# Chlumsky/msdfgen

Hardware: AMD Instinct MI355X
Metric: MSDF glyphs/sec (64x64, fp32) (higher is better)
Workload: dtype f64

## Files before the change

msdfgen_amd/csrc/msdf_cull.hpp:

```cpp
#pragma once

#include <string.h>
#include "msdf_device.hpp"

namespace msdfhip {

#define MSDF_CULL_SLACK (1.+1e-6)

MSDF_HD double cullUpperDistance(const EdgeRec &e, V2 c) {
    const V2 a = c-ld(e.p0), b = c-ld(e.pe), m = c-ld(e.mid);
    const double da = dot(a, a), db = dot(b, b), dm = dot(m, m);
    return sqrt(cmin(cmin(da, db), dm));
}

MSDF_HD float cullNearestSample2(const EdgeRec &e, V2 c) {
    const V2 a = c-ld(e.p0), b = c-ld(e.pe), m = c-ld(e.mid);
    return (float) cmin(cmin(dot(a, a), dot(b, b)), dot(m, m));
}
MSDF_HD float cullBumpUp(float f) {
    unsigned bits;
    memcpy(&bits, &f, sizeof(bits));
    if (bits < 0x7f800000u)
        ++bits;
    memcpy(&f, &bits, sizeof(bits));
    return f;
}
MSDF_HD float cullUpperFromSample2(float sample2) {
    return cullBumpUp(sqrtf(cullBumpUp(sample2)));
}

MSDF_HD double cullLowerDistance2(const EdgeRec &e, V2 c) {
    const double dx = cmax(cmax(e.lo[0]-c.x, c.x-e.hi[0]), 0.);
    const double dy = cmax(cmax(e.lo[1]-c.y, c.y-e.hi[1]), 0.);
    return dx*dx+dy*dy;
}

template <bool PERP>
MSDF_HD bool cullEdgeSurvives(const EdgeRec &e, V2 c, double r, double Umax) {
    const double R = r*MSDF_CULL_SLACK;
    const double reach = (Umax+R)*MSDF_CULL_SLACK;
    const double beyond = reach+R;
    if (!(cullLowerDistance2(e, c) > beyond*beyond))
        return true;
    if (PERP) {
        const V2 ap = c-ld(e.p0), aDir = ld(e.aDirN);
        const bool outsideA = dot(ap, ld(e.na))+R <= 0 || -dot(ap, aDir)+R <= 0;
        if (!outsideA && !(fabs(cross(ap, aDir))-R > reach))
            return true;
        const V2 bp = c-ld(e.pe), bDir = ld(e.bDirN);
        const bool outsideB = -dot(bp, ld(e.nb))+R <= 0 || dot(bp, bDir)+R <= 0;
        if (!outsideB && !(fabs(cross(bp, bDir))-R > reach))
            return true;
    }
    return false;
}

MSDF_HD unsigned cullOrderKeyOfSample2(float d2, int slot) {
    unsigned bits;
    memcpy(&bits, &d2, sizeof(bits));
    if (!(bits < 0x7f800000u))
        bits = 0x7f7ffff0u;
    return (bits&~15u)|(unsigned) (slot&15);
}
MSDF_HD unsigned cullOrderKey(const EdgeRec &e, V2 c, int slot) { return cullOrderKeyOfSample2(cullNearestSample2(e, c), slot); }
#define MSDF_CULL_KEY_DROPPED 0x7f800000u
#define MSDF_CULL_KEY_DROPPED_SEGMENTED 0xfffffff0u

template <int SEL>
MSDF_HD int cullMask(const EdgeRec &e) { return SEL <= 2 ? 1 : (e.color&7); }

}
```

msdfgen_amd/csrc/msdf_device.hpp:

```cpp
#pragma once

#include <stdint.h>
#include <stddef.h>
#include <math.h>
#include <float.h>

#if defined(__HIPCC__)
#define MSDF_HD __host__ __device__ inline
#define MSDF_NOINLINE __attribute__((noinline))
#define MSDF_NOUNROLL _Pragma("clang loop unroll(disable)")
#define MSDF_UNROLL _Pragma("unroll")
#if defined(__HIP_DEVICE_COMPILE__)
#define MSDF_UNIFORM(x) __builtin_amdgcn_readfirstlane(x)
#else
#define MSDF_UNIFORM(x) (x)
#endif
#else
#define MSDF_HD inline
#define MSDF_NOINLINE
#define MSDF_NOUNROLL
#define MSDF_UNROLL
#define MSDF_UNIFORM(x) (x)
#endif

#define MSDF_UNLIKELY(x) __builtin_expect(!!(x), 0)

#include "msdf_measure.hpp"

namespace msdfhip {

#if defined(__HIP_DEVICE_COMPILE__)
#define MSDF_WAVE_ANY(pred) (__any((int) (pred)) != 0)
#else
#define MSDF_WAVE_ANY(pred) (pred)
#endif


enum : int32_t {
    REC_A_ZERO = 1,
    REC_B_ZERO = 2,
    REC_NORMED = 4,
    REC_CORNER = 8,
    REC_FASTDIV = 16
};

struct V2 { double x, y; };

struct alignas(128) EdgeRec {
    double lo[2];
    double hi[2];
    double p0[2];
    double pe[2];
    double na[2];
    double nb[2];
    double aDirN[2];
    double bDirN[2];
    double ab[2];
    double k[6];
    double br[2];
    double ep0[2];
    double ep1[2];
    double e0dot;
    double e1dot;
    double rcp[4];
    double p1[2];
    double as_[2];
    double p2[2];
    double mid[2];
    int32_t type;
    int32_t color;
    int32_t flags;
    int32_t contour;
    double pad_[2];

    MSDF_HD V2 Lo() const; MSDF_HD V2 Hi() const; MSDF_HD V2 P0() const; MSDF_HD V2 PE() const; MSDF_HD V2 P1() const;
    MSDF_HD V2 NA() const; MSDF_HD V2 NB() const; MSDF_HD V2 ADirN() const; MSDF_HD V2 BDirN() const;
    MSDF_HD V2 AB() const; MSDF_HD V2 BR() const; MSDF_HD V2 AS() const; MSDF_HD V2 EP0() const; MSDF_HD V2 EP1() const;
    MSDF_HD double E0dot() const { return e0dot; }
    MSDF_HD double E1dot() const { return e1dot; }
    MSDF_HD double K(int i) const { return k[i]; }
    MSDF_HD double Rcp(int i) const { return rcp[i]; }
    MSDF_HD int Type() const { return type; }
    MSDF_HD int Color() const { return color; }
    MSDF_HD int Flags() const { return flags; }
};
static_assert(sizeof(EdgeRec) == 384, "EdgeRec layout");
static_assert(offsetof(EdgeRec, na) == 0x40 && offsetof(EdgeRec, ab) == 0x80 && offsetof(EdgeRec, br) == 0xc0 && offsetof(EdgeRec, rcp) == 0x100 &&
              offsetof(EdgeRec, p2) == 0x140 && offsetof(EdgeRec, type) == 0x160, "EdgeRec blocks");

MSDF_HD V2 mk(double x, double y) { V2 r; r.x = x; r.y = y; return r; }
MSDF_HD V2 operator+(V2 a, V2 b) { return mk(a.x+b.x, a.y+b.y); }
MSDF_HD V2 operator-(V2 a, V2 b) { return mk(a.x-b.x, a.y-b.y); }
MSDF_HD V2 operator-(V2 a) { return mk(-a.x, -a.y); }
MSDF_HD V2 operator*(double a, V2 b) { return mk(a*b.x, a*b.y); }
MSDF_HD double dot(V2 a, V2 b) { return a.x*b.x+a.y*b.y; }
MSDF_HD double cross(V2 a, V2 b) { return a.x*b.y-a.y*b.x; }

#if defined(__HIP_DEVICE_COMPILE__)
__device__ inline double leanSqrtCore(double x) {
    const double y = __builtin_amdgcn_rsq(x);
    double g = x*y;
    double h = y*.5;
    const double r = __builtin_fma(-h, g, .5);
    g = __builtin_fma(g, r, g);
    h = __builtin_fma(h, r, h);
    double d = __builtin_fma(-g, g, x);
    g = __builtin_fma(d, h, g);
    d = __builtin_fma(-g, g, x);
    return __builtin_fma(d, h, g);
}
__device__ inline double msdfSqrt(double x) {
    const unsigned hi = (unsigned) __double2hiint(x);
    if (__any((int) (hi-0x10000000u >= 0x7ff00000u-0x10000000u)))
        return sqrt(x);
    return leanSqrtCore(x);
}
#else
MSDF_HD double msdfSqrt(double x) { return sqrt(x); }
#endif
MSDF_HD double vlen(V2 a) { return msdfSqrt(a.x*a.x+a.y*a.y); }
MSDF_HD V2 ld(const double *p) { return mk(p[0], p[1]); }
MSDF_HD V2 EdgeRec::Lo() const { return ld(lo); }
MSDF_HD V2 EdgeRec::Hi() const { return ld(hi); }
MSDF_HD V2 EdgeRec::P0() const { return ld(p0); }
MSDF_HD V2 EdgeRec::PE() const { return ld(pe); }
MSDF_HD V2 EdgeRec::P1() const { return ld(p1); }
MSDF_HD V2 EdgeRec::NA() const { return ld(na); }
MSDF_HD V2 EdgeRec::NB() const { return ld(nb); }
MSDF_HD V2 EdgeRec::ADirN() const { return ld(aDirN); }
MSDF_HD V2 EdgeRec::BDirN() const { return ld(bDirN); }
MSDF_HD V2 EdgeRec::AB() const { return ld(ab); }
MSDF_HD V2 EdgeRec::BR() const { return ld(br); }
MSDF_HD V2 EdgeRec::AS() const { return ld(as_); }
MSDF_HD V2 EdgeRec::EP0() const { return ld(ep0); }
MSDF_HD V2 EdgeRec::EP1() const { return ld(ep1); }

MSDF_HD V2 normalize(V2 a, bool allowZero) {
    double len = vlen(a);
    if (len != 0)
        return mk(a.x/len, a.y/len);
    return mk(0, allowZero ? 0. : 1.);
}

MSDF_HD V2 normalizeLen(V2 a, double len, bool allowZero) {
    if (len != 0)
        return mk(a.x/len, a.y/len);
    return mk(0, allowZero ? 0. : 1.);
}

MSDF_HD V2 orthonormalFalse(V2 a) {
    double len = vlen(a);
    if (len != 0)
        return mk(a.y/len, -a.x/len);
    return mk(0, -1.);
}

MSDF_HD V2 mixv(V2 a, V2 b, double w) { return (1.-w)*a+w*b; }
MSDF_HD double nonZeroSign(double n) { return n > 0 ? 1. : -1.; }
MSDF_HD double dmin(double a, double b) { return b < a ? b : a; }
MSDF_HD double dmax(double a, double b) { return a < b ? b : a; }
MSDF_HD double cmax(double a, double b) { return __builtin_fmax(a, b); }
MSDF_HD double cmin(double a, double b) { return __builtin_fmin(a, b); }
MSDF_HD double median(double a, double b, double c) { return dmax(dmin(a, b), dmin(dmax(a, b), c)); }
MSDF_HD float fmin_(float a, float b) { return b < a ? b : a; }
MSDF_HD float fmax_(float a, float b) { return a < b ? b : a; }
MSDF_HD float medianf(float a, float b, float c) { return fmax_(fmin_(a, b), fmin_(fmax_(a, b), c)); }
MSDF_HD float med3Max(float a, float b) {
// ... 446 lines not shown
    if (o.neg > b.neg)
        b.neg = o.neg;
    if (o.pos < b.pos)
        b.pos = o.pos;
}

MSDF_HD double pbCompute(const PB &b) {
    double m = b.td < 0 ? b.neg : b.pos;
    if (pbHasNear(b) && fabs(b.perp) < fabs(m))
        m = b.perp;
    return m;
}

MSDF_HD bool getPerpendicularDistance(double &distance, V2 ep, V2 edgeDir) {
    double ts = dot(ep, edgeDir);
    if (ts > 0) {
        double perp = cross(ep, edgeDir);
        if (fabs(perp) < fabs(distance)) {
            distance = perp;
            return true;
        }
    }
    return false;
}

template <int SEL> struct SelTraits { enum { NPB = SEL == 1 ? 0 : SEL == 2 ? 1 : 3, NCH = SEL <= 2 ? 1 : SEL }; };

template <int SEL>
struct Selector {
    SD m;
    PB c[(int) SelTraits<SEL>::NPB > 0 ? (int) SelTraits<SEL>::NPB : 1];
    int idx[(int) SelTraits<SEL>::NPB > 0 ? (int) SelTraits<SEL>::NPB : 1];
};

template <int SEL>
MSDF_HD void selInit(Selector<SEL> &s) {
    s.m.d = -DBL_MAX, s.m.dot = 0;
    s.idx[0] = 0x7fffffff;
    for (int i = 0; i < (int) SelTraits<SEL>::NPB; ++i) {
        pbInit(s.c[i]);
        s.idx[i] = 0x7fffffff;
    }
}

MSDF_HD bool sdReplaces(SD sd, int idx, SD cur, int curIdx) {
    return sdLess(sd, cur) || (fabs(sd.d) == fabs(cur.d) && sd.dot == cur.dot && idx < curIdx);
}
MSDF_HD bool sdReplacesWave(SD sd, int idx, SD cur, int curIdx) {
    const double a = fabs(sd.d), b = fabs(cur.d);
    bool r = a < b;
    if (MSDF_WAVE_ANY(a == b))
        r = r || (a == b && (sd.dot < cur.dot || (sd.dot == cur.dot && idx < curIdx)));
    return r;
}

template <int SEL, class Rec>
MSDF_HD void selAddEdge(Selector<SEL> &s, const Rec &e, int idx, V2 o) {
    if (SEL == 1) {
        double dummy;
        SD sd = signedDistance(e, o, dummy);
        if (sdReplacesWave(sd, idx, s.m, s.idx[0]))
            s.m = sd, s.idx[0] = idx;
        return;
    }
    const int mask = SEL == 2 ? 1 : (e.Color()&7);
    if (!mask)
        return;
    double param;
    SD sd = signedDistance(e, o, param);
    bool nearer[(int) SelTraits<SEL>::NPB > 0 ? (int) SelTraits<SEL>::NPB : 1];
    bool any = false;
    for (int i = 0; i < (int) SelTraits<SEL>::NPB; ++i) {
        SD cur = { s.c[i].td, s.c[i].tdot };
        nearer[i] = (mask&(1<<i)) && sdReplacesWave(sd, idx, cur, s.idx[i]);
        any = any || nearer[i];
    }
    if (any) {
        SD conv = sd;
        distanceToPerpendicular(e, conv, o, param);
        for (int i = 0; i < (int) SelTraits<SEL>::NPB; ++i)
            if (nearer[i])
                s.c[i].td = sd.d, s.c[i].tdot = sd.dot, s.c[i].perp = conv.d, s.idx[i] = idx;
    }
    V2 ap = o-e.P0();
    V2 bp = o-e.PE();
    double add = dot(ap, e.NA());
    double bdd = -dot(bp, e.NB());
    if (add > 0) {
        double pd = sd.d;
        if (getPerpendicularDistance(pd, ap, -e.ADirN())) {
            pd = -pd;
            for (int i = 0; i < (int) SelTraits<SEL>::NPB; ++i)
                pbAddPerpIf(s.c[i], pd, (mask&(1<<i)) != 0);
        }
    }
    if (bdd > 0) {
        double pd = sd.d;
        if (getPerpendicularDistance(pd, bp, e.BDirN())) {
            for (int i = 0; i < (int) SelTraits<SEL>::NPB; ++i)
                pbAddPerpIf(s.c[i], pd, (mask&(1<<i)) != 0);
        }
    }
}

template <int SEL, class Rec>
MSDF_HD bool selEdgeRelevantBox(const Selector<SEL> &s, const Rec &e, V2 o, double &bound2) {
    if (SEL == 1)
        bound2 = s.m.d*s.m.d;
    else {
        const int mask = SEL == 2 ? 1 : (e.Color()&7);
        bound2 = -1;
        if (!mask)
            return false;
        bound2 = 0;
        double t = 0;
        for (int i = 0; i < (int) SelTraits<SEL>::NPB; ++i)
            t = cmax(t, fabs(s.c[i].td)*((mask&(1<<i)) ? 1. : 0.));
        bound2 = t*t;
    }
    bound2 *= 1+1e-9;
    const double dx = cmax(cmax(e.Lo().x-o.x, o.x-e.Hi().x), 0.);
    const double dy = cmax(cmax(e.Lo().y-o.y, o.y-e.Hi().y), 0.);
    return !(dx*dx+dy*dy > bound2);
}
template <int SEL, class Rec>
MSDF_HD bool selEdgeRelevantWedges(const Rec &e, V2 o, double bound2) {
    if (SEL >= 2) {
        const V2 ap = o-e.P0(), aDir = e.ADirN();
        if (dot(ap, e.NA()) > 0 && dot(ap, -aDir) > 0) {
            const double perp = cross(ap, aDir);
            if (!(perp*perp > bound2))
                return true;
        }
        const V2 bp = o-e.PE(), bDir = e.BDirN();
        if (-dot(bp, e.NB()) > 0 && dot(bp, bDir) > 0) {
            const double perp = cross(bp, bDir);
            if (!(perp*perp > bound2))
                return true;
        }
    }
    return false;
}
template <int SEL, class Rec>
MSDF_HD bool selEdgeRelevant(const Selector<SEL> &s, const Rec &e, V2 o) {
    double bound2;
    return selEdgeRelevantBox(s, e, o, bound2) || selEdgeRelevantWedges<SEL>(e, o, bound2);
}

template <int SEL>
MSDF_HD void selMerge(Selector<SEL> &s, const Selector<SEL> &o) {
    if (SEL == 1) {
        if (sdLess(o.m, s.m))
            s.m = o.m;
        return;
    }
    for (int i = 0; i < (int) SelTraits<SEL>::NPB; ++i)
        pbMergeWave(s.c[i], o.c[i]);
}

template <int SEL>
MSDF_HD void selDistance(const Selector<SEL> &s, double *out) {
    if (SEL == 1) {
        out[0] = s.m.d;
        return;
    }
    for (int i = 0; i < (int) SelTraits<SEL>::NPB; ++i)
        out[i] = pbCompute(s.c[i]);
    if (SEL == 4) {
        SD t = { s.c[0].td, s.c[0].tdot };
        SD g = { s.c[SEL == 4 ? 1 : 0].td, s.c[SEL == 4 ? 1 : 0].tdot };
        SD b = { s.c[SEL == 4 ? 2 : 0].td, s.c[SEL == 4 ? 2 : 0].tdot };
        if (sdLess(g, t))
            t = g;
        if (sdLess(b, t))
            t = b;
        out[SEL == 4 ? 3 : 0] = t.d;
    }
}

template <int SEL>
MSDF_HD double resolve(const double *d) {
    return SEL >= 3 ? median(d[0], d[SEL >= 3 ? 1 : 0], d[SEL >= 3 ? 2 : 0]) : d[0];
}


struct EdgesAll {
    const int32_t *coff;
    MSDF_HD int begin(int c) const { return coff[c]-coff[0]; }
    MSDF_HD int end(int c) const { return coff[c+1]-coff[0]; }
    MSDF_HD int at(int k) const { return k; }
};
struct EdgesCulled {
    const int *cstart;
    const int *list;
    MSDF_HD int begin(int c) const { return MSDF_UNIFORM(cstart[c]); }
    MSDF_HD int end(int c) const { return MSDF_UNIFORM(cstart[c+1]); }
    MSDF_HD int at(int k) const { return list ? MSDF_UNIFORM(list[k])&0xfffff : k; }
};

template <int SEL, class Edges>
MSDF_HD void selAddContourSerial(Selector<SEL> &sel, const EdgeRec *rec, const Edges &edges, int c, V2 o) {
    const int e = edges.end(c);
    for (int k = edges.begin(c); k < e; ++k) {
        const int i = edges.at(k);
        if (MSDF_WAVE_ANY(selEdgeRelevant(sel, rec[i], o)))
            selAddEdge(sel, rec[i], i, o);
    }
}
template <int SEL> MSDF_HD void selAddContour(Selector<SEL> &sel, const EdgeRec *rec, const EdgesAll &edges, int c, V2 o) { selAddContourSerial(sel, rec, edges, c, o); }
template <int SEL> MSDF_HD void selAddContour(Selector<SEL> &sel, const EdgeRec *rec, const EdgesCulled &edges, int c, V2 o) { selAddContourSerial(sel, rec, edges, c, o); }

struct NoTeam {
    template <int SEL> MSDF_HD bool afterWalk(Selector<SEL> &) const { return true; }
    MSDF_HD bool isHelper() const { return false; }
};

template <int SEL>
MSDF_HD void selMergePartial(Selector<SEL> &a, const Selector<SEL> &b) {
    if (SEL == 1) {
        if (sdReplaces(b.m, b.idx[0], a.m, a.idx[0]))
            a.m = b.m, a.idx[0] = b.idx[0];
// ... 291 lines not shown
```

msdfgen_amd/csrc/msdf_kernels.hpp:

```cpp
#pragma once

#include <hip/hip_runtime.h>
#include "msdf_device.hpp"
#include "msdf_prep.hpp"
#include "msdf_ec.hpp"
#include "msdf_ec_fast.hpp"
#include "msdf_cull.hpp"
#include "msdf_scanline.hpp"
#include "msdf_shapeprep.hpp"
#include "msdf_frame.hpp"
#include "msdf_legacy.hpp"
#include "../../include/msdfgen_hip.h"

namespace msdfhip {

#ifndef MSDF_DISTANCE_WAVES_PER_SIMD
#define MSDF_DISTANCE_WAVES_PER_SIMD 4
#endif
constexpr int TILE = 8;
constexpr int WAVE = 64;
constexpr int REC_DOUBLES = sizeof(EdgeRec)/sizeof(double);

struct BatchView {
    int nGlyphs;
// ... 131 lines not shown

__device__ inline unsigned nextItem(unsigned *counters, unsigned total, int &steal) {
    const unsigned x = blockIdx.x&7u;
    while (steal < 8) {
        const unsigned xx = (x+(unsigned) steal)&7u;
        unsigned k = 0;
        if (threadIdx.x == 0)
            k = atomicAdd(&counters[xx], 1u);
        k = (unsigned) __builtin_amdgcn_readfirstlane((int) k);
        const unsigned b = k*8u+xx;
        if (b < total)
            return b;
        ++steal;
    }
    return ~0u;
}

__device__ inline Xform loadXform(const MsdfHipGlyph &gd) {
    Xform t;
    t.sx = gd.xf[0], t.sy = gd.xf[1], t.tx = gd.xf[2], t.ty = gd.xf[3];
    t.mapScale = gd.xf[4], t.mapTranslate = gd.xf[5];
    return t;
}

__device__ inline void stageRecords(double *dst, const EdgeRec *src, int n) {
    const double *s = reinterpret_cast<const double *>(src);
    const int total = n*REC_DOUBLES;
    for (int i = threadIdx.x; i < total; i += blockDim.x)
        dst[i] = s[i];
}


__device__ inline void waveSync() {
    __builtin_amdgcn_fence(__ATOMIC_RELEASE, "wavefront");
    __builtin_amdgcn_wave_barrier();
    __builtin_amdgcn_fence(__ATOMIC_ACQUIRE, "wavefront");
}

__device__ inline float waveMinNonNegative(float v) {
    int x = __float_as_int(v);
    const int inf = 0x7f800000;
#define MSDF_DPP_MIN(ctrl, rowmask) { const int y = __builtin_amdgcn_update_dpp(inf, x, ctrl, rowmask, 0xf, false); x = y < x ? y : x; }
    MSDF_DPP_MIN(0x111, 0xf)
    MSDF_DPP_MIN(0x112, 0xf)
    MSDF_DPP_MIN(0x114, 0xf)
    MSDF_DPP_MIN(0x118, 0xf)
    MSDF_DPP_MIN(0x142, 0xa)
    MSDF_DPP_MIN(0x143, 0xc)
#undef MSDF_DPP_MIN
    return __int_as_float(__builtin_amdgcn_readlane(x, 63));
}

__device__ inline float floatAbove(double d) {
    float f = (float) d;
    if ((double) f < d)
        f = __int_as_float(__float_as_int(f)+1);
    return f;
}

__device__ inline float rowMinNonNegative(float v, int lane) {
    int x = __float_as_int(v);
    const int inf = 0x7f800000;
#define MSDF_DPP_MIN(ctrl) { const int y = __builtin_amdgcn_update_dpp(inf, x, ctrl, 0xf, 0xf, false); x = y < x ? y : x; }
    MSDF_DPP_MIN(0x111)
    MSDF_DPP_MIN(0x112)
    MSDF_DPP_MIN(0x114)
    MSDF_DPP_MIN(0x118)
#undef MSDF_DPP_MIN
    return __int_as_float(__shfl(x, lane|15));
}

__device__ inline int rowRank(unsigned key) {
    int rank = 0;
#define MSDF_DPP_ROR(n) rank += (unsigned) __builtin_amdgcn_update_dpp((int) key, (int) key, 0x120+n, 0xf, 0xf, false) < key ? 1 : 0;
    MSDF_DPP_ROR(1) MSDF_DPP_ROR(2) MSDF_DPP_ROR(3) MSDF_DPP_ROR(4) MSDF_DPP_ROR(5) MSDF_DPP_ROR(6) MSDF_DPP_ROR(7) MSDF_DPP_ROR(8)
    MSDF_DPP_ROR(9) MSDF_DPP_ROR(10) MSDF_DPP_ROR(11) MSDF_DPP_ROR(12) MSDF_DPP_ROR(13) MSDF_DPP_ROR(14) MSDF_DPP_ROR(15)
#undef MSDF_DPP_ROR
    return rank;
}

typedef double d8 __attribute__((ext_vector_type(8)));

enum { ENTRY_INDEX_BITS = 20, ENTRY_INDEX_MASK = (1<<ENTRY_INDEX_BITS)-1 };
__device__ inline unsigned packEntry(int i, const EdgeRec &e) {
    return (unsigned) (i&ENTRY_INDEX_MASK)|(unsigned) e.type<<20|(unsigned) (e.color&7)<<22|(unsigned) (e.flags&7)<<25|(unsigned) ((e.flags>>4)&1)<<28;
}

struct EdgeRegs {
    d8 r0, r1, e0, e1, e2;
    unsigned meta;
    __device__ V2 Lo() const { return mk(r0[0], r0[1]); }
    __device__ V2 Hi() const { return mk(r0[2], r0[3]); }
    __device__ V2 P0() const { return mk(r0[4], r0[5]); }
    __device__ V2 PE() const { return mk(r0[6], r0[7]); }
    __device__ V2 NA() const { return mk(r1[0], r1[1]); }
    __device__ V2 NB() const { return mk(r1[2], r1[3]); }
    __device__ V2 ADirN() const { return mk(r1[4], r1[5]); }
    __device__ V2 BDirN() const { return mk(r1[6], r1[7]); }
    __device__ V2 AB() const { return mk(e0[0], e0[1]); }
    __device__ double K(int i) const { return e0[2+i]; }
    __device__ V2 BR() const { return mk(e1[0], e1[1]); }
    __device__ V2 EP0() const { return mk(e1[2], e1[3]); }
    __device__ V2 EP1() const { return mk(e1[4], e1[5]); }
    __device__ double E0dot() const { return e1[6]; }
    __device__ double E1dot() const { return e1[7]; }
    __device__ double Rcp(int i) const { return e2[i]; }
    __device__ V2 P1() const { return mk(e2[4], e2[5]); }
    __device__ V2 AS() const { return mk(e2[6], e2[7]); }
    __device__ int Type() const { return (int) (meta>>20)&3; }
    __device__ int Color() const { return (int) (meta>>22)&7; }
    __device__ int Flags() const { return (int) ((meta>>25)&7)|(int) ((meta>>28)&1)<<4; }
};
static_assert(REC_A_ZERO == 1 && REC_B_ZERO == 2 && REC_NORMED == 4 && REC_FASTDIV == 16, "packEntry / EdgeRegs::Flags");

__device__ inline EdgeRegs loadEdgeRegs(const EdgeRec *rp, int i) {
    const d8 *blocks = reinterpret_cast<const d8 *>(rp);
    EdgeRegs r;
    r.r0 = blocks[0], r.r1 = blocks[1], r.e0 = blocks[2], r.e1 = blocks[3], r.e2 = blocks[4];
    r.meta = packEntry(i, *rp);
    return r;
}

struct WindingMasks {
    unsigned long long pos, neg;
    const int8_t *mem;
    __device__ int operator[](int c) const {
        if (c < 64)
            return (int) ((pos>>c)&1ull)-(int) ((neg>>c)&1ull);
        return mem[c];
    }
};

struct PackedSurvivors {
    const int *cstart;
    const int *list;
    int total;
    int first, step;
    __device__ int begin(int c) const { return MSDF_UNIFORM(cstart[c]); }
    __device__ int end(int c) const { return MSDF_UNIFORM(cstart[c+1]); }
};
struct EdgesCulledPacked : PackedSurvivors, WaitCounters { };

template <int SEL>
__device__ inline void selAddContour(Selector<SEL> &sel, const EdgeRec *rec, const EdgesCulledPacked &edges, int c, V2 o) {
    const int e = edges.end(c);
    int k = edges.begin(c)+edges.first;
    if (k >= e)
        return;
    unsigned cur = (unsigned) MSDF_UNIFORM(edges.list[k]);
    MSDF_NOUNROLL
    for (; k < e; k += edges.step) {
        const EdgeRec *rp = rec+(cur&ENTRY_INDEX_MASK);
        EdgeRegs r;
        r.meta = cur;
        unsigned nextV;
        const unsigned nextAddr = (unsigned) (size_t) (edges.list+k+edges.step);
        const unsigned long long t0 = profNow(edges);
        asm volatile("ds_read_b32 %0, %4\n\ts_load_dwordx16 %1, %5, 0x0\n\ts_load_dwordx16 %2, %5, 0x40\n\ts_load_dwordx16 %3, %5, 0x80\n\ts_waitcnt lgkmcnt(0)"
                     : "=v"(nextV), "=&s"(r.r0), "=&s"(r.r1), "=&s"(r.e0) : "v"(nextAddr), "s"(rp));
        const unsigned long long t1 = profNow(edges);
        profBatch(edges, t1-t0);
        const unsigned next = k+edges.step < edges.total ? (unsigned) __builtin_amdgcn_readfirstlane((int) nextV) : cur;
        double bound2;
        bool relevant = MSDF_WAVE_ANY(selEdgeRelevantBox(sel, r, o, bound2));
        if (SEL >= 2 && !relevant)
            relevant = MSDF_WAVE_ANY(selEdgeRelevantWedges<SEL>(r, o, bound2));
        const unsigned long long t2 = profNow(edges);
        profAdd(edges, PROF_RELEVANCE, t2-t1);
        if (relevant) {
            if (r.Type() >= 2)
                asm volatile("s_load_dwordx16 %0, %2, 0xc0\n\ts_load_dwordx16 %1, %2, 0x100\n\ts_waitcnt lgkmcnt(0)" : "=&s"(r.e1), "=&s"(r.e2) : "s"(rp));
            const unsigned long long t3 = profNow(edges);
            if (r.Type() >= 2)
                profAdd(edges, PROF_CURVE_BATCH, t3-t2), profAdd(edges, PROF_CURVE_BATCH+1, 1);
            selAddEdge(sel, r, (int) (cur&ENTRY_INDEX_MASK), o);
            profPin(edges, sel.c[0].td);
            profAdd(edges, PROF_EVAL, profNow(edges)-t3), profAdd(edges, PROF_EVAL+1, 1);
        }
        cur = next;
    }
}

typedef int i4 __attribute__((ext_vector_type(4)));
struct EdgesAllBatched {
    const int32_t *coff;
    __device__ int begin(int c) const { return coff[c]-coff[0]; }
    __device__ int end(int c) const { return coff[c+1]-coff[0]; }
};

template <int SEL>
__device__ inline void selAddContour(Selector<SEL> &sel, const EdgeRec *rec, const EdgesAllBatched &edges, int c, V2 o) {
    const int e = MSDF_UNIFORM(edges.end(c));
    MSDF_NOUNROLL
    for (int i = MSDF_UNIFORM(edges.begin(c)); i < e; ++i) {
        const EdgeRec *rp = rec+i;
        EdgeRegs r;
        i4 words;
        asm volatile("s_load_dwordx16 %0, %4, 0x0\n\ts_load_dwordx16 %1, %4, 0x40\n\ts_load_dwordx16 %2, %4, 0x80\n\ts_load_dwordx4 %3, %4, 0x160\n\ts_waitcnt lgkmcnt(0)"
                     : "=&s"(r.r0), "=&s"(r.r1), "=&s"(r.e0), "=&s"(words) : "s"(rp));
        r.meta = (unsigned) (i&ENTRY_INDEX_MASK)|(unsigned) words[0]<<20|(unsigned) (words[1]&7)<<22|(unsigned) (words[2]&7)<<25|(unsigned) ((words[2]>>4)&1)<<28;
        double bound2;
        bool relevant = MSDF_WAVE_ANY(selEdgeRelevantBox(sel, r, o, bound2));
        if (SEL >= 2 && !relevant)
            relevant = MSDF_WAVE_ANY(selEdgeRelevantWedges<SEL>(r, o, bound2));
        if (relevant) {
            if (r.Type() >= 2)
                asm volatile("s_load_dwordx16 %0, %2, 0xc0\n\ts_load_dwordx16 %1, %2, 0x100\n\ts_waitcnt lgkmcnt(0)" : "=&s"(r.e1), "=&s"(r.e2) : "s"(rp));
            selAddEdge(sel, r, i, o);
        }
    }
}

struct EdgesGrid {
    const int32_t *coff;
    int slice, S;
    __device__ int begin(int c) const { return coff[c]-coff[0]; }
    __device__ int end(int c) const { return coff[c+1]-coff[0]; }
};

__device__ inline void selAddContour(Selector<2> &sel, const EdgeRec *rec, const EdgesGrid &edges, int c, V2 o) {
    Selector<2> mine;
    selInit(mine);
    const int e = MSDF_UNIFORM(edges.end(c));
    MSDF_NOUNROLL
    for (int i = MSDF_UNIFORM(edges.begin(c))+edges.slice; i < e; i += edges.S) {
        const EdgeRegs r = loadEdgeRegs(rec+i, i);
        selAddEdge(mine, r, i, o);
    }
    MSDF_NOUNROLL
    for (int off = 1; off < edges.S; off <<= 1) {
        Selector<2> other;
        selInit(other);
        PB &m = mine.c[0], &t = other.c[0];
        t.td = __shfl_xor(m.td, off), t.tdot = __shfl_xor(m.tdot, off), t.perp = __shfl_xor(m.perp, off);
        t.neg = __shfl_xor(m.neg, off), t.pos = __shfl_xor(m.pos, off);
        other.idx[0] = __shfl_xor(mine.idx[0], off);
        selMergePartial(mine, other);
    }
    selMergePartial(sel, mine);
}

template <bool OVERLAP, class Wind>
struct PsdfQueryGrid {
    const EdgeRec *rec;
    const int32_t *coff;
    Wind windings;
    int C, slice, S;
    double *res;
// ... 111 lines not shown
        for (int q = 0; q < TPW_; ++q) {
            const int tileQ = wk.tile*TPW_+q;
            some = some || (tileQ < tilesPerGlyph && (tileQ%tilesX)*TILE < boxW && (tileQ/tilesX)*TILE < boxH);
        }
        if (!some) {
            if (!persistent)
                return;
            continue;
        }
    }
    const int c0 = knownContours >= 0 ? 0 : MSDF_UNIFORM(batch.glyphContourOffsets[wk.g]), C = knownContours >= 0 ? knownContours : MSDF_UNIFORM(batch.glyphContourOffsets[wk.g+1])-c0;
    const int32_t *coff = batch.contourOffsets+c0;
    const int e0 = knownContours >= 0 ? 0 : MSDF_UNIFORM(coff[0]);
    const int lane = TEAM > 1 ? (int) (threadIdx.x&(WAVE-1)) : (int) threadIdx.x;
    const EdgeRec *rec = batch.recs+e0;

    double *res = GRES ? gres+(size_t) blockId*gresStride : smem;
    int *lists = reinterpret_cast<int *>(smem+(OVERLAP && !GRES ? (size_t) C*NCH*WAVE : 0));
    int *cstarts = lists+(size_t) TPW*maxEdges;

    const MsdfHipGlyph gd = glyphs[wk.g];
    const Xform t = loadXform(gd);
    WindingMasks wind;
    wind.mem = batch.windings+c0;
    if (OVERLAP) {
        const int w = lane < C ? (int) wind.mem[lane] : 0;
        wind.pos = __ballot(w > 0), wind.neg = __ballot(w < 0);
    }
    WaitProbe probe;
    WaitCounters sums;
    probe.begin(sums);

    const double rsx = 1/t.sx, rsy = 1/t.sy;
    const bool fastXf = divSafe(t.sx) && divSafe(t.sy);
    const double hx = (.5*TILE-.5)*fabs(rsx), hy = (.5*TILE-.5)*fabs(rsy);
    const double tr = sqrt(hx*hx+hy*hy);
    if (TEAM == 1 || teamRank == 0) {
        const int q = lane/ROW, col = lane%ROW;
        const int tileQ = wk.tile*TPW+q;
        const bool tileInGrid = tileQ < tilesPerGlyph;
        const int txq = tileQ%tilesX, tyq = tileQ/tilesX;
        const bool tileValid = tileInGrid && (!SIZED || (txq*TILE < boxW && tyq*TILE < boxH));
        const V2 tc = mk((txq*TILE+.5*TILE)*rsx-t.tx, (tyq*TILE+.5*TILE)*rsy-t.ty);
        int *list = lists+(size_t) q*maxEdges, *cstart = cstarts+(size_t) q*(C+1);
        int nSurv = 0;
        double U[3] = { DBL_MAX, DBL_MAX, DBL_MAX };
        const int nE = knownEdges >= 0 ? knownEdges : coff[C]-e0;
        probe.headerLanded(nE+(int) gd.flip);
        unsigned *bounds = (GRES || !OVERLAP ? reinterpret_cast<unsigned *>(cstarts+(size_t) TPW*(C+1)) : reinterpret_cast<unsigned *>(smem))+(size_t) q*C*3;
        if (OVERLAP) {
            for (int k = col; k < C*3; k += ROW)
                bounds[k] = 0x7f800000u;
            waveSync();
        }
        for (int base = 0; base < nE; base += ROW) {
            const int i = base+col;
            float sample2 = 0;
            int mask = 0;
            if (i < nE && tileValid) {
                mask = cullMask<SEL>(rec[i]);
                if (mask || !OVERLAP)
                    sample2 = cullNearestSample2(rec[i], tc);
                list[i] = __float_as_int(sample2);
            }
            const float ubf = cullUpperFromSample2(sample2);
            if (OVERLAP) {
                if (mask) {
                    unsigned *mine = bounds+(size_t) (rec[i].contour-c0)*3;
                    for (int ch = 0; ch < (SEL <= 2 ? 1 : 3); ++ch)
                        if ((mask>>ch)&1)
                            atomicMin(mine+ch, (unsigned) __float_as_int(ubf));
                }
            } else
                for (int ch = 0; ch < (SEL <= 2 ? 1 : 3); ++ch)
                    U[ch] = dmin(U[ch], (double) (TPW == 1 ? waveMinNonNegative((mask>>ch)&1 ? ubf : __int_as_float(0x7f800000))
                                                           : rowMinNonNegative((mask>>ch)&1 ? ubf : __int_as_float(0x7f800000), lane)));
        }
        if (OVERLAP)
            waveSync();
        probe.passADone(sums);
        for (int base = 0; base < nE; base += ROW) {
            const int i = base+col;
            bool keep = false;
            int c = 0;
            float sample2 = 0;
            if (i < nE) {
                if (tileValid)
                    sample2 = __int_as_float(list[i]);
                c = rec[i].contour-c0;
                const int mask = cullMask<SEL>(rec[i]);
                if (mask && tileValid) {
                    double umax = 0;
                    for (int ch = 0; ch < (SEL <= 2 ? 1 : 3); ++ch)
                        if ((mask>>ch)&1)
                            umax = dmax(umax, OVERLAP ? (double) __int_as_float((int) bounds[(size_t) c*3+ch]) : U[ch]);
                    keep = cullEdgeSurvives<(SEL >= 2)>(rec[i], tc, tr, umax);
                }
            }
            const int segment = c-__shfl(c, lane&~15);
            const bool wideRow = ((__ballot(i < nE && segment > 15)>>(lane&~15))&0xffffull) != 0;
            unsigned key = MSDF_CULL_KEY_DROPPED_SEGMENTED|(unsigned) (col&15);
            if (keep) {
                const unsigned d = (cullOrderKeyOfSample2(sample2, 0)>>3)&0x0ffffff0u;
                key = wideRow ? (unsigned) (col&15) : ((unsigned) segment<<28)|(d < 0x0ffffff0u ? d : 0x0fffffe0u)|(unsigned) (col&15);
            }
            const int rank = rowRank(key);
            const unsigned long long ballot = __ballot(keep);
            const unsigned long long rowBallot = TPW == 1 ? ballot : (ballot>>(ROW*q))&0xffffull;
            const int before = TPW == 1 ? __popcll(ballot&((1ull<<(col&~15))-1ull)) : 0;
            if (keep)
                list[nSurv+before+rank] = (int) packEntry(i, rec[i]);
            if (i < nE && coff[c]-e0 == i) {
                const int at = nSurv+__popcll(rowBallot&((1ull<<col)-1ull));
                cstart[c] = at;
                for (int cc = c-1; cc >= 0 && coff[cc]-e0 == i; --cc)
                    cstart[cc] = at;
            }
            nSurv += __popcll(rowBallot);
        }
        for (int c = col; c < C; c += ROW)
            if (coff[c]-e0 == nE)
                cstart[c] = nSurv;
        if (col == 0)
            cstart[C] = nSurv;
    }
    waveSync();
    if (TEAM > 1)
        __syncthreads();
    probe.phase1Done();

    if (TPW == 1 && knownContours >= 0) {
        const int total = MSDF_UNIFORM(cstarts[C]);
        for (int base = 0; base < total; base += WAVE) {
            const int entry = base+lane < total ? lists[base+lane] : 0;
            const int n = total-base < WAVE ? total-base : WAVE;
            for (int k = 0; k < n; k += 4) {
                const EdgeRec *r0 = rec+(__builtin_amdgcn_readlane(entry, k)&ENTRY_INDEX_MASK);
                const EdgeRec *r1 = rec+(__builtin_amdgcn_readlane(entry, k+1 < n ? k+1 : k)&ENTRY_INDEX_MASK);
                const EdgeRec *r2 = rec+(__builtin_amdgcn_readlane(entry, k+2 < n ? k+2 : k)&ENTRY_INDEX_MASK);
                const EdgeRec *r3 = rec+(__builtin_amdgcn_readlane(entry, k+3 < n ? k+3 : k)&ENTRY_INDEX_MASK);
                int sink;
                asm volatile("s_load_dword %0, %1, 0x0\n\ts_load_dword %0, %1, 0x40\n\ts_load_dword %0, %1, 0x80\n\ts_load_dword %0, %1, 0xc0\n\ts_load_dword %0, %1, 0x100\n\t"
                             "s_load_dword %0, %2, 0x0\n\ts_load_dword %0, %2, 0x40\n\ts_load_dword %0, %2, 0x80\n\ts_load_dword %0, %2, 0xc0\n\ts_load_dword %0, %2, 0x100\n\t"
                             "s_load_dword %0, %3, 0x0\n\ts_load_dword %0, %3, 0x40\n\ts_load_dword %0, %3, 0x80\n\ts_load_dword %0, %3, 0xc0\n\ts_load_dword %0, %3, 0x100\n\t"
                             "s_load_dword %0, %4, 0x0\n\ts_load_dword %0, %4, 0x40\n\ts_load_dword %0, %4, 0x80\n\ts_load_dword %0, %4, 0xc0\n\ts_load_dword %0, %4, 0x100\n\t"
                             "s_waitcnt lgkmcnt(0)" : "=&s"(sink) : "s"(r0), "s"(r1), "s"(r2), "s"(r3));
            }
        }
    }

    MSDF_NOUNROLL
    for (int q = 0; q < TPW; ++q) {
        const int tile = wk.tile*TPW+q;
        if (tile >= tilesPerGlyph)
            break;
        const int tx = tile%tilesX, ty = tile/tilesX;
        const int x = tx*TILE+(lane&(TILE-1)), y = ty*TILE+(lane>>3);
        if (x >= boxW || y >= boxH)
            continue;
        const V2 p = fastXf ? mk(divExact(x+.5, t.sx, rsx)-t.tx, divExact(y+.5, t.sy, rsy)-t.ty)
                            : unproject(t, mk(x+.5, y+.5));
        EdgesCulledPacked edges;
        edges.total = MSDF_UNIFORM(cstarts[(size_t) q*(C+1)+C]);
        const unsigned long long tTile0 = profReset(edges);
        edges.cstart = cstarts+(size_t) q*(C+1);
        edges.list = lists+(size_t) q*maxEdges;
        edges.first = teamRank, edges.step = TEAM;
        TeamExchange<TEAM> team;
        team.x = teamXchg, team.lane = lane, team.rank = teamRank;
        double d[NCH];
        if (OVERLAP) {
            EdgesCulled cold;
            cold.cstart = edges.cstart, cold.list = edges.list;
            if (TEAM > 1)
                shapeDistanceOverlapSplit<SEL>(rec, edges, cold, wind, C, p, res+lane, WAVE, d, team);
            else
                shapeDistanceOverlapSplit<SEL>(rec, edges, cold, wind, C, p, res+lane, WAVE, d);
        } else if (TEAM > 1)
            shapeDistanceSimple<SEL>(rec, edges, C, p, d, team);
        else
            shapeDistanceSimple<SEL>(rec, edges, C, p, d);
        if (TEAM > 1 && teamRank != 0)
            continue;
        int laneAfter = lane;
#if defined(__HIP_DEVICE_COMPILE__)
        asm volatile("" : "+v"(laneAfter));
#endif
        const int xo = tx*TILE+(laneAfter&(TILE-1)), yo = ty*TILE+(laneAfter>>3);
        const int yn = gd.flip ? boxH-1-yo : yo;
        float *px = toScratch ? dst+(SIZED ? (size_t) wk.g*width*height+(size_t) yn*boxW+xo : ((size_t) wk.g*height+yn)*width+xo)*NCH
                              : dst+gd.out_offset+(ptrdiff_t) gd.row_stride*yn+(ptrdiff_t) NCH*xo;
        for (int ch = 0; ch < NCH; ++ch) {
            __builtin_nontemporal_store(mapDistance(t, d[ch]), &px[ch]);
        }
// ... 1560 lines not shown
```

Baseline: 1.953 million.

## Carry per-tile wedge-outside flags into packed entries to skip endpoint wedge work

During tile culling, the code now computes once per tile whether each surviving edge's endpoint wedges A and B lie entirely outside the tile's radius, and stores those two bits in spare high bits of the packed entry word. The per-pixel evaluation reads the bits to skip the endpoint perpendicular-distance updates and the wedge relevance tests, and it skips the wedge test entirely when both wedges are outside. This moves per-pixel wedge checks to a per-tile conservative check, at the cost of two more packed bits and a small branch per edge.

```diff
diff --git a/msdfgen_amd/csrc/msdf_cull.hpp b/msdfgen_amd/csrc/msdf_cull.hpp
--- a/msdfgen_amd/csrc/msdf_cull.hpp
+++ b/msdfgen_amd/csrc/msdf_cull.hpp
@@ -35,8 +35,18 @@
     return dx*dx+dy*dy;
 }
 
+enum { CULL_OUTSIDE_A = 1, CULL_OUTSIDE_B = 2 };
+MSDF_HD int cullWedgeOutside(const EdgeRec &e, V2 c, double r) {
+    const double R = r*MSDF_CULL_SLACK;
+    const V2 ap = c-ld(e.p0), aDir = ld(e.aDirN);
+    const bool outsideA = dot(ap, ld(e.na))+R <= 0 || -dot(ap, aDir)+R <= 0;
+    const V2 bp = c-ld(e.pe), bDir = ld(e.bDirN);
+    const bool outsideB = -dot(bp, ld(e.nb))+R <= 0 || dot(bp, bDir)+R <= 0;
+    return (outsideA ? (int) CULL_OUTSIDE_A : 0)|(outsideB ? (int) CULL_OUTSIDE_B : 0);
+}
+
 template <bool PERP>
-MSDF_HD bool cullEdgeSurvives(const EdgeRec &e, V2 c, double r, double Umax) {
+MSDF_HD bool cullEdgeSurvives(const EdgeRec &e, V2 c, double r, double Umax, int outside) {
     const double R = r*MSDF_CULL_SLACK;
     const double reach = (Umax+R)*MSDF_CULL_SLACK;
     const double beyond = reach+R;
@@ -44,15 +54,17 @@
         return true;
     if (PERP) {
         const V2 ap = c-ld(e.p0), aDir = ld(e.aDirN);
-        const bool outsideA = dot(ap, ld(e.na))+R <= 0 || -dot(ap, aDir)+R <= 0;
-        if (!outsideA && !(fabs(cross(ap, aDir))-R > reach))
+        if (!(outside&CULL_OUTSIDE_A) && !(fabs(cross(ap, aDir))-R > reach))
             return true;
         const V2 bp = c-ld(e.pe), bDir = ld(e.bDirN);
-        const bool outsideB = -dot(bp, ld(e.nb))+R <= 0 || dot(bp, bDir)+R <= 0;
-        if (!outsideB && !(fabs(cross(bp, bDir))-R > reach))
+        if (!(outside&CULL_OUTSIDE_B) && !(fabs(cross(bp, bDir))-R > reach))
             return true;
     }
     return false;
+}
+template <bool PERP>
+MSDF_HD bool cullEdgeSurvives(const EdgeRec &e, V2 c, double r, double Umax) {
+    return cullEdgeSurvives<PERP>(e, c, r, Umax, PERP ? cullWedgeOutside(e, c, r) : 0);
 }
 
 MSDF_HD unsigned cullOrderKeyOfSample2(float d2, int slot) {
diff --git a/msdfgen_amd/csrc/msdf_device.hpp b/msdfgen_amd/csrc/msdf_device.hpp
--- a/msdfgen_amd/csrc/msdf_device.hpp
+++ b/msdfgen_amd/csrc/msdf_device.hpp
@@ -83,6 +83,8 @@
     MSDF_HD int Type() const { return type; }
     MSDF_HD int Color() const { return color; }
     MSDF_HD int Flags() const { return flags; }
+    MSDF_HD bool OutsideA() const { return false; }
+    MSDF_HD bool OutsideB() const { return false; }
 };
 static_assert(sizeof(EdgeRec) == 384, "EdgeRec layout");
 static_assert(offsetof(EdgeRec, na) == 0x40 && offsetof(EdgeRec, ab) == 0x80 && offsetof(EdgeRec, br) == 0xc0 && offsetof(EdgeRec, rcp) == 0x100 &&
@@ -695,23 +697,27 @@
             if (nearer[i])
                 s.c[i].td = sd.d, s.c[i].tdot = sd.dot, s.c[i].perp = conv.d, s.idx[i] = idx;
     }
-    V2 ap = o-e.P0();
-    V2 bp = o-e.PE();
-    double add = dot(ap, e.NA());
-    double bdd = -dot(bp, e.NB());
-    if (add > 0) {
-        double pd = sd.d;
-        if (getPerpendicularDistance(pd, ap, -e.ADirN())) {
-            pd = -pd;
-            for (int i = 0; i < (int) SelTraits<SEL>::NPB; ++i)
-                pbAddPerpIf(s.c[i], pd, (mask&(1<<i)) != 0);
-        }
-    }
-    if (bdd > 0) {
-        double pd = sd.d;
-        if (getPerpendicularDistance(pd, bp, e.BDirN())) {
-            for (int i = 0; i < (int) SelTraits<SEL>::NPB; ++i)
-                pbAddPerpIf(s.c[i], pd, (mask&(1<<i)) != 0);
+    if (!e.OutsideA()) {
+        V2 ap = o-e.P0();
+        double add = dot(ap, e.NA());
+        if (add > 0) {
+            double pd = sd.d;
+            if (getPerpendicularDistance(pd, ap, -e.ADirN())) {
+                pd = -pd;
+                for (int i = 0; i < (int) SelTraits<SEL>::NPB; ++i)
+                    pbAddPerpIf(s.c[i], pd, (mask&(1<<i)) != 0);
+            }
+        }
+    }
+    if (!e.OutsideB()) {
+        V2 bp = o-e.PE();
+        double bdd = -dot(bp, e.NB());
+        if (bdd > 0) {
+            double pd = sd.d;
+            if (getPerpendicularDistance(pd, bp, e.BDirN())) {
+                for (int i = 0; i < (int) SelTraits<SEL>::NPB; ++i)
+                    pbAddPerpIf(s.c[i], pd, (mask&(1<<i)) != 0);
+            }
         }
     }
 }
@@ -739,17 +745,21 @@
 template <int SEL, class Rec>
 MSDF_HD bool selEdgeRelevantWedges(const Rec &e, V2 o, double bound2) {
     if (SEL >= 2) {
-        const V2 ap = o-e.P0(), aDir = e.ADirN();
-        if (dot(ap, e.NA()) > 0 && dot(ap, -aDir) > 0) {
-            const double perp = cross(ap, aDir);
-            if (!(perp*perp > bound2))
-                return true;
-        }
-        const V2 bp = o-e.PE(), bDir = e.BDirN();
-        if (-dot(bp, e.NB()) > 0 && dot(bp, bDir) > 0) {
-            const double perp = cross(bp, bDir);
-            if (!(perp*perp > bound2))
-                return true;
+        if (!e.OutsideA()) {
+            const V2 ap = o-e.P0(), aDir = e.ADirN();
+            if (dot(ap, e.NA()) > 0 && dot(ap, -aDir) > 0) {
+                const double perp = cross(ap, aDir);
+                if (!(perp*perp > bound2))
+                    return true;
+            }
+        }
+        if (!e.OutsideB()) {
+            const V2 bp = o-e.PE(), bDir = e.BDirN();
+            if (-dot(bp, e.NB()) > 0 && dot(bp, bDir) > 0) {
+                const double perp = cross(bp, bDir);
+                if (!(perp*perp > bound2))
+                    return true;
+            }
         }
     }
     return false;
diff --git a/msdfgen_amd/csrc/msdf_kernels.hpp b/msdfgen_amd/csrc/msdf_kernels.hpp
--- a/msdfgen_amd/csrc/msdf_kernels.hpp
+++ b/msdfgen_amd/csrc/msdf_kernels.hpp
@@ -237,8 +237,10 @@
 typedef double d8 __attribute__((ext_vector_type(8)));
 
 enum { ENTRY_INDEX_BITS = 20, ENTRY_INDEX_MASK = (1<<ENTRY_INDEX_BITS)-1 };
-__device__ inline unsigned packEntry(int i, const EdgeRec &e) {
-    return (unsigned) (i&ENTRY_INDEX_MASK)|(unsigned) e.type<<20|(unsigned) (e.color&7)<<22|(unsigned) (e.flags&7)<<25|(unsigned) ((e.flags>>4)&1)<<28;
+enum { ENTRY_OUTSIDE_SHIFT = 29 };
+__device__ inline unsigned packEntry(int i, const EdgeRec &e, int outside = 0) {
+    return (unsigned) (i&ENTRY_INDEX_MASK)|(unsigned) e.type<<20|(unsigned) (e.color&7)<<22|(unsigned) (e.flags&7)<<25|(unsigned) ((e.flags>>4)&1)<<28|
+           (unsigned) (outside&3)<<ENTRY_OUTSIDE_SHIFT;
 }
 
 struct EdgeRegs {
@@ -265,7 +267,10 @@
     __device__ int Type() const { return (int) (meta>>20)&3; }
     __device__ int Color() const { return (int) (meta>>22)&7; }
     __device__ int Flags() const { return (int) ((meta>>25)&7)|(int) ((meta>>28)&1)<<4; }
+    __device__ bool OutsideA() const { return ((meta>>ENTRY_OUTSIDE_SHIFT)&CULL_OUTSIDE_A) != 0; }
+    __device__ bool OutsideB() const { return ((meta>>ENTRY_OUTSIDE_SHIFT)&CULL_OUTSIDE_B) != 0; }
 };
+static_assert(CULL_OUTSIDE_A == 1 && CULL_OUTSIDE_B == 2 && ENTRY_OUTSIDE_SHIFT+2 <= 31 && ENTRY_OUTSIDE_SHIFT > 28, "packEntry / EdgeRegs::OutsideA, OutsideB");
 static_assert(REC_A_ZERO == 1 && REC_B_ZERO == 2 && REC_NORMED == 4 && REC_FASTDIV == 16, "packEntry / EdgeRegs::Flags");
 
 __device__ inline EdgeRegs loadEdgeRegs(const EdgeRec *rp, int i) {
@@ -318,7 +323,7 @@
         const unsigned next = k+edges.step < edges.total ? (unsigned) __builtin_amdgcn_readfirstlane((int) nextV) : cur;
         double bound2;
         bool relevant = MSDF_WAVE_ANY(selEdgeRelevantBox(sel, r, o, bound2));
-        if (SEL >= 2 && !relevant)
+        if (SEL >= 2 && !relevant && !(r.OutsideA() && r.OutsideB()))
             relevant = MSDF_WAVE_ANY(selEdgeRelevantWedges<SEL>(r, o, bound2));
         const unsigned long long t2 = profNow(edges);
         profAdd(edges, PROF_RELEVANCE, t2-t1);
@@ -596,7 +601,7 @@
         for (int base = 0; base < nE; base += ROW) {
             const int i = base+col;
             bool keep = false;
-            int c = 0;
+            int c = 0, outside = 0;
             float sample2 = 0;
             if (i < nE) {
                 if (tileValid)
@@ -608,7 +613,9 @@
                     for (int ch = 0; ch < (SEL <= 2 ? 1 : 3); ++ch)
                         if ((mask>>ch)&1)
                             umax = dmax(umax, OVERLAP ? (double) __int_as_float((int) bounds[(size_t) c*3+ch]) : U[ch]);
-                    keep = cullEdgeSurvives<(SEL >= 2)>(rec[i], tc, tr, umax);
+                    if (SEL >= 2)
+                        outside = cullWedgeOutside(rec[i], tc, tr);
+                    keep = cullEdgeSurvives<(SEL >= 2)>(rec[i], tc, tr, umax, outside);
                 }
             }
             const int segment = c-__shfl(c, lane&~15);
@@ -623,7 +630,7 @@
             const unsigned long long rowBallot = TPW == 1 ? ballot : (ballot>>(ROW*q))&0xffffull;
             const int before = TPW == 1 ? __popcll(ballot&((1ull<<(col&~15))-1ull)) : 0;
             if (keep)
-                list[nSurv+before+rank] = (int) packEntry(i, rec[i]);
+                list[nSurv+before+rank] = (int) packEntry(i, rec[i], outside);
             if (i < nE && coff[c]-e0 == i) {
                 const int at = nSurv+__popcll(rowBallot&((1ull<<col)-1ull));
                 cstart[c] = at;
```

New measurement: 2.050 million (median of 6 runs). 1.05x the previous value.
